# gooey-audio/libgooey

Measured on NVIDIA B200. Metric: voice-samples/sec, higher is better.
Workload: dtype f32

## Files before the change

libgooey_b200/csrc/kernels.cuh:

```cuda
#pragma once
#include <cuda_runtime.h>
#include "voices2.cuh"

namespace gd {

constexpr int TILE = 32;

template <class S> __device__ __forceinline__ void load_words(S& s, const uint32_t* base, int slot, int n_pad, int w0) {
  constexpr int W = sizeof(S) / 4;
  uint32_t* w = reinterpret_cast<uint32_t*>(&s);
#pragma unroll
  for (int i = 0; i < W; i++) w[i] = base[(size_t)(w0 + i) * n_pad + slot];
}
template <class S> __device__ __forceinline__ void store_words(const S& s, uint32_t* base, int slot, int n_pad, int w0) {
  constexpr int W = sizeof(S) / 4;
  const uint32_t* w = reinterpret_cast<const uint32_t*>(&s);
#pragma unroll
  for (int i = 0; i < W; i++) base[(size_t)(w0 + i) * n_pad + slot] = w[i];
}

struct KickV {
  using State = KickState; using Ctl = KickCtl; using Aud = KickAud; using Span = KickSpan;
  static constexpr bool FAST = true; static constexpr int NPL = KICK_PLANES;
  struct Run { KickDer d; int j_act; };
  static __device__ __forceinline__ float tick(State& s, const double* tt, const RateCtx& rc) { return kick_tick(s, tt, rc); }
  static __device__ __forceinline__ void slow_event(State& s, const VoiceEvent& e, const double* tt, const RateCtx&) {
    uint32_t r = 0; kick_event(s.c, e, tt, r); kick_span_begin(s.a, s.c, r);
  }
  static __device__ __forceinline__ bool settled(const Ctl& c) { return params_settled<K_NP>(c.cur, c.tgt); }
  static __device__ __forceinline__ void event(Ctl& c, const VoiceEvent& e, const double* tt, uint32_t& r) { kick_event(c, e, tt, r); }
  static __device__ __forceinline__ void plan(Ctl& c, uint32_t r, const double* tt, int ja, int jb, Span& sp) { kick_plan(c, r, tt, ja, jb, sp); }
  static __device__ __forceinline__ int front_end(const Span& sp) { return sp.j_act; }
  static __device__ __forceinline__ void front(const Span& sp, double now, uint32_t, float sr, float* o) {
    KickFront f = sp.d.drive <= 8.0f ? kick_front<true>(sp.c, sp.d, now, sr) : kick_front<false>(sp.c, sp.d, now, sr);
    o[0] = f.p1; o[1] = f.raw_click; o[2] = f.ne; o[3] = f.amp;
  }
  static __device__ __forceinline__ void span_begin(Aud& a, const Span& sp, Run& r, float) { kick_span_begin(a, sp.c, sp.resets); r.d = sp.d; r.j_act = sp.j_act; }
  static __device__ __forceinline__ void span_resume(const Span& sp, Run& r) { r.d = sp.d; r.j_act = sp.j_act; }
  static __device__ __forceinline__ bool wants_planes(const Aud&, const Run& r, int j) { return j < r.j_act; }
  static __device__ __forceinline__ bool is_active(const Aud&, const Run& r, int j) { return j < r.j_act; }
  static __device__ __forceinline__ float back(Aud& a, const Run& r, int j, const float* p, const RateCtx& rc) {
    if (j >= r.j_act) return 0.0f;
    KickFront f; f.p1 = p[0]; f.raw_click = p[1]; f.ne = p[2]; f.amp = p[3];
    return kick_back(a, r.d, f, rc);
  }
};
struct SnareV {
  using State = SnareState; using Ctl = SnareCtl; using Aud = SnareAud; using Span = SnareSpan;
  static constexpr bool FAST = true; static constexpr int NPL = SNARE_PLANES;
  struct Run { SnareDer d; int j_act; };
  static __device__ __forceinline__ float tick(State& s, const double* tt, const RateCtx& rc) { return snare_tick(s, tt, rc); }
  static __device__ __forceinline__ void slow_event(State& s, const VoiceEvent& e, const double* tt, const RateCtx&) {
    uint32_t r = 0; snare_event(s.c, e, tt, r); snare_span_begin(s.a, s.c, r);
  }
  static __device__ __forceinline__ bool settled(const Ctl& c) { return params_settled<S_NP>(c.cur, c.tgt); }
  static __device__ __forceinline__ void event(Ctl& c, const VoiceEvent& e, const double* tt, uint32_t& r) { snare_event(c, e, tt, r); }
  static __device__ __forceinline__ void plan(Ctl& c, uint32_t r, const double* tt, int ja, int jb, Span& sp) { snare_plan(c, r, tt, ja, jb, sp); }
  static __device__ __forceinline__ int front_end(const Span& sp) { return sp.j_act; }
  static __device__ __forceinline__ void front(const Span& sp, double now, uint32_t, float sr, float* o) {
    SnareFront f = snare_front<true>(sp.c, sp.d, now, sr);
    o[0] = f.tonal_out; o[1] = f.raw_noise; o[2] = f.cne; o[3] = f.crack_out; o[4] = f.amp;
  }
  static __device__ __forceinline__ void span_begin(Aud& a, const Span& sp, Run& r, float) { snare_span_begin(a, sp.c, sp.resets); r.d = sp.d; r.j_act = sp.j_act; }
  static __device__ __forceinline__ void span_resume(const Span& sp, Run& r) { r.d = sp.d; r.j_act = sp.j_act; }
  static __device__ __forceinline__ bool wants_planes(const Aud&, const Run& r, int j) { return j < r.j_act; }
  static __device__ __forceinline__ bool is_active(const Aud&, const Run& r, int j) { return j < r.j_act; }
  static __device__ __forceinline__ float back(Aud& a, const Run& r, int j, const float* p, const RateCtx& rc) {
    if (j >= r.j_act) return 0.0f;
    SnareFront f; f.tonal_out = p[0]; f.raw_noise = p[1]; f.cne = p[2]; f.crack_out = p[3]; f.amp = p[4];
    return snare_back(a, r.d, f, rc);
  }
};
struct HatV {
  using State = HatState; using Ctl = HatCtl; using Aud = HatAud; using Span = HatSpan;
  static constexpr bool FAST = true; static constexpr int NPL = HAT_PLANES;
  struct Run { HatDer d; int j_env; float env_final; };
  static __device__ __forceinline__ float tick(State& s, const double* tt, const RateCtx& rc) { return hat_tick(s, tt, rc); }
  static __device__ __forceinline__ void slow_event(State& s, const VoiceEvent& e, const double* tt, const RateCtx&) {
    uint32_t r = 0; hat_event(s.c, e, tt, r); hat_span_begin(s.a, s.c, r);
  }
  static __device__ __forceinline__ bool settled(const Ctl& c) { return params_settled<H_NP>(c.cur, c.tgt); }
  static __device__ __forceinline__ void event(Ctl& c, const VoiceEvent& e, const double* tt, uint32_t& r) { hat_event(c, e, tt, r); }
  static __device__ __forceinline__ void plan(Ctl& c, uint32_t r, const double* tt, int ja, int jb, Span& sp) { hat_plan(c, r, tt, ja, jb, sp); }
  static __device__ __forceinline__ int front_end(const Span& sp) { return sp.j_env < sp.j1 ? sp.j_env : sp.j1; }
  static __device__ __forceinline__ void front(const Span& sp, double now, uint32_t, float sr, float* o) { o[0] = hat_front(sp.c, sp.d, now, sr).env; }
  static __device__ __forceinline__ void span_begin(Aud& a, const Span& sp, Run& r, float) { hat_span_begin(a, sp.c, sp.resets); span_resume(sp, r); }
  static __device__ __forceinline__ void span_resume(const Span& sp, Run& r) { r.d = sp.d; r.j_env = sp.j_env; r.env_final = sp.env_final; }
  static __device__ __forceinline__ bool wants_planes(const Aud& a, const Run& r, int j) { return a.active && j < r.j_env; }
  static __device__ __forceinline__ bool is_active(const Aud& a, const Run&, int) { return a.active != 0; }
  static __device__ __forceinline__ float back(Aud& a, const Run& r, int j, const float* p, const RateCtx& rc) {
    if (!a.active) return 0.0f;
    HatFront f; f.env = j < r.j_env ? p[0] : r.env_final;
    return hat_back(a, r.d, f, j >= r.j_env, rc);
  }
};
struct TomV {
  using State = TomState; using Ctl = TomCtl; using Aud = TomAud; using Span = TomSpan;
  static constexpr bool FAST = true; static constexpr int NPL = TOM_PLANES;
  struct Run { TomDer d; int j_env; float env_final; };
  static __device__ __forceinline__ float tick(State& s, const double* tt, const RateCtx& rc) { return tom_tick(s, tt, rc); }
  static __device__ __forceinline__ void slow_event(State& s, const VoiceEvent& e, const double* tt, const RateCtx& rc) {
    uint32_t r = 0; tom_event(s.c, e, tt, r); tom_span_begin(s.a, s.c.mem_q_scale, s.c.mem_gain_scale, s.c.mem_dirty, r, rc.sr); s.c.mem_dirty = 0;
  }
  static __device__ __forceinline__ bool settled(const Ctl&) { return true; }
  static __device__ __forceinline__ void event(Ctl& c, const VoiceEvent& e, const double* tt, uint32_t& r) { tom_event(c, e, tt, r); }
  static __device__ __forceinline__ void plan(Ctl& c, uint32_t r, const double* tt, int ja, int jb, Span& sp) { tom_plan(c, r, tt, ja, jb, sp); }
  static __device__ __forceinline__ int front_end(const Span& sp) { return sp.d.membrane > 0.0f ? sp.j1 : (sp.j_env < sp.j1 ? sp.j_env + 1 : sp.j1); }
  static __device__ __forceinline__ void front(const Span& sp, double now, uint32_t k, float, float* o) {
    TomFront f = tom_front(sp.c, sp.d, now, k); o[0] = f.env; o[1] = f.noise; o[2] = f.rnd;
  }
  static __device__ __forceinline__ void span_begin(Aud& a, const Span& sp, Run& r, float sr) {
    tom_span_begin(a, sp.mem_q_scale, sp.mem_gain_scale, sp.mem_dirty, sp.resets, sr); span_resume(sp, r);
  }
// ... 64 lines not shown
      if (!((row_mask >> r) & 1u)) continue;
      const long long row = rows ? (long long)rows[r] : (long long)(row0 + r);
      if (lane < nf) out[row * stride + f0 + lane] = tile[r * 33 + lane];
    }
  }
}
__device__ __forceinline__ void load_tile_rows(float* tile , const float* plane, int pitch, int row0, int n_rows, int c0, int lane) {
  const int c = (lane & 7) * 4;
#pragma unroll
  for (int k = 0; k < 8; k++) {
    const int r = k * 4 + (lane >> 3);
    if (r < n_rows) {
      const float4 v = *reinterpret_cast<const float4*>(plane + (size_t)(row0 + r) * pitch + c0 + c);
      float* dst = tile + r * 33 + c;
      dst[0] = v.x; dst[1] = v.y; dst[2] = v.z; dst[3] = v.w;
    }
  }
}

__device__ __forceinline__ void load_tile_rows_any(float* tile , const float* plane, long long pitch, int row0, int n_rows, int c0, int nf, int lane) {
  for (int r = 0; r < n_rows; r++)
    if (lane < nf) tile[r * 33 + lane] = plane[(long long)(row0 + r) * pitch + c0 + lane];
}

template <class V, int BLOCK>
__global__ void __launch_bounds__(BLOCK) slow_kernel(const VoiceLaunch L) {
  __shared__ float tiles[BLOCK / 32][TILE * 33];
  const int v = blockIdx.x * BLOCK + threadIdx.x;
  const int lane = threadIdx.x & 31;
  const int warp = threadIdx.x >> 5;
// ... 144 lines not shown
#pragma unroll
        for (int q = 0; q < V::NPL; q++) p[q] = tl[q][lane * 33 + jj];
        tout[lane * 33 + jj] = V::back(a, run, j, p, L.rc);
      }
    }
    __syncwarp();
    store_tile_voice_major(tout, L.out, L.stride, L.row0 + warp_v0, L.rows ? L.rows + warp_v0 : nullptr, row_mask, L.chunk0 + f0, nf, lane);
    __syncwarp();
  }
  if (mine) {
    store_words(a, L.state, sv, L.n_pad, WC);
    L.span_cursor[v] = cur;
  }
}

#ifndef GOOEY_OWN_KERNELS_TU
__global__ void __launch_bounds__(64) lfo_kernel(LfoStream* __restrict__ streams, int n, float* __restrict__ planes, long long pitch, int frames) {
  const int i = blockIdx.x * blockDim.x + threadIdx.x;
  if (i >= n) return;
  LfoStream s = streams[i];
  float* out = s.plane >= 0 ? planes + (long long)s.plane * pitch : nullptr;
  for (int f = 0; f < frames; f++) {
    const float value = gm::g_sinf(s.phase * 2.0f * PI_F);
    s.phase += s.inc;
    if (s.phase >= 1.0f) s.phase -= 1.0f;
    if (out) out[f] = s.offset + (value * s.amount);
  }
  streams[i].phase = s.phase;
}
#endif
// ... 3 lines not shown
```

libgooey_b200/csrc/pool.cuh:

```cuda
#pragma once
#include <algorithm>
#include <atomic>
#include <map>
#include <type_traits>
#include <set>
#include <mutex>
#include "device_rt.h"
#include "wave.cuh"
#include "coop.cuh"
#include "gran_wave.cuh"
#include "bass_wave.cuh"
#include "poly_wave.cuh"
#include "../../include/gooey_batch.h"

namespace gh {

extern std::atomic<uint64_t> g_launches;

struct KernelStat { uint64_t launches = 0; double ms = 0.0; double voice_frames = 0.0; };
std::map<std::string, KernelStat>& kernel_stats();
std::mutex& kernel_stats_mutex();

__global__ void scatter_words_kernel(uint32_t* __restrict__ dst, long long cap, const uint32_t* __restrict__ src, const uint32_t* __restrict__ slots,
                                     int n, int words) {
// ... 135 lines not shown
  std::lock_guard<std::mutex> lk(mu);
  if (done.insert({dev, (const void*)kernel}).second)
    GH_CUDA(cudaFuncSetAttribute((const void*)kernel, cudaFuncAttributePreferredSharedMemoryCarveout, (int)cudaSharedmemCarveoutMaxShared));
}
#define GH_LAUNCH(kernel, grid, block, stream, ...) do { same_carveout(kernel); kernel<<<grid, block, 0, stream>>>(__VA_ARGS__); } while (0)

constexpr int CHUNK_FRAMES = 8192;
template <class V> struct TypeRunner {
  using State = typename V::State;
  Pool<State> pool;
  std::vector<uint32_t> slots, rows, ev_begin, span_off;
  std::vector<gd::VoiceEvent> ev_flat;
  std::vector<gd::ModRoute> routes_flat; std::vector<uint32_t> route_begin;
  DevBuf<gd::ModRoute> d_routes; DevBuf<uint32_t> d_route_begin;
  const float* mod_planes = nullptr; long long mod_pitch = 0; int mod_frame0 = 0;
  DevBuf<uint32_t> d_slots, d_rows, d_ev_begin, d_span_off, d_n_spans, d_span_cursor;
  DevBuf<gd::VoiceEvent> d_events;
  DevBuf<uint8_t> d_mode, d_spans;
  DevBuf<float> d_planes[2];
  cudaStream_t sB = nullptr, sC = nullptr, sS = nullptr;
  cudaEvent_t evA = nullptr, evB[2] = {nullptr, nullptr}, evC[2] = {nullptr, nullptr}, evDoneC = nullptr, evDoneS = nullptr;
  std::vector<cudaEvent_t> evT0, evT1;
  std::vector<double> timed_units;
  std::vector<cudaEvent_t> evChunk;
  int launched_chunks = 0;
  int timed_launches = 0;
  const char* backend_name = "back_kernel";
  static int chunk_of(int frames) { return std::min(CHUNK_FRAMES, (frames + 31) & ~31); }
  void wait_chunk(cudaStream_t s, int i) {
    if (n() == 0) return;
    if (launched_chunks == 0) { GH_CUDA(cudaStreamWaitEvent(s, evDoneC, 0)); return; }
    GH_CUDA(cudaStreamWaitEvent(s, evDoneS, 0));
    GH_CUDA(cudaStreamWaitEvent(s, evChunk[std::min(i, std::abs(launched_chunks) - 1)], 0));
  }

  int n() const { return (int)slots.size(); }
// ... 2 lines not shown
  void add(uint32_t slot, uint32_t out_row, const std::vector<gd::VoiceEvent>& events, const std::vector<gd::ModRoute>* routes = nullptr) {
    slots.push_back(slot); rows.push_back(out_row);
    if (routes) routes_flat.insert(routes_flat.end(), routes->begin(), routes->end());
    route_begin.push_back((uint32_t)routes_flat.size());
    uint32_t distinct = 0, last = 0xffffffffu;
    for (const auto& e : events) { if (e.frame != last) { distinct++; last = e.frame; } }
    ev_flat.insert(ev_flat.end(), events.begin(), events.end());
    ev_begin.push_back((uint32_t)ev_flat.size());
    span_off.push_back(span_off.back() + distinct + 1);
  }
  void ensure_streams() {
    if (sC) return;
    GH_CUDA(cudaStreamCreateWithFlags(&sB, cudaStreamNonBlocking));
    GH_CUDA(cudaStreamCreateWithFlags(&sC, cudaStreamNonBlocking));
    GH_CUDA(cudaStreamCreateWithFlags(&sS, cudaStreamNonBlocking));
    cudaEvent_t* evs[] = {&evA, &evB[0], &evB[1], &evC[0], &evC[1], &evDoneC, &evDoneS};
    for (auto e : evs) GH_CUDA(cudaEventCreateWithFlags(e, cudaEventDisableTiming));
  }
  ~TypeRunner() {
    cudaEvent_t evs[] = {evA, evB[0], evB[1], evC[0], evC[1], evDoneC, evDoneS};
    for (auto e : evs) if (e) cudaEventDestroy(e);
    for (auto e : evChunk) cudaEventDestroy(e);
    for (auto e : evT0) cudaEventDestroy(e);
    for (auto e : evT1) cudaEventDestroy(e);
    if (sB) cudaStreamDestroy(sB);
    if (sC) cudaStreamDestroy(sC);
    if (sS) cudaStreamDestroy(sS);
  }
  void collect_stats() {
    const char* name = backend_name;
    const int timed = V::FAST ? launched_chunks : timed_launches;
    if (timed <= 0) return;
    std::lock_guard<std::mutex> lk(kernel_stats_mutex());
    KernelStat& k = kernel_stats()[name];
    for (int i = 0; i < timed; i++) {
      float ms = 0.0f;
      if (cudaEventElapsedTime(&ms, evT0[i], evT1[i]) != cudaSuccess) { cudaGetLastError(); continue; }
      k.launches++; k.ms += ms; k.voice_frames += timed_units[i];
    }
    if (V::FAST) launched_chunks = -launched_chunks;
    else timed_launches = 0;
  }
// ... 13 lines not shown
    memset(&L, 0, sizeof L);
    L.state = pool.d.p; L.n = cnt; L.n_pad = pool.cap;
    L.slots = d_slots.p; L.rows = d_rows.p; L.row0 = 0;
    L.events = d_events.p; L.ev_begin = d_ev_begin.p; L.tt = tt; L.frames = frames; L.out = out; L.stride = stride; L.rc = rc;
    const bool modulated = !routes_flat.empty() && mod_planes;
    if (modulated) {
      d_routes.upload(routes_flat.data(), routes_flat.size(), sC);
      d_route_begin.upload(route_begin.data(), route_begin.size(), sC);
      L.routes = d_routes.p; L.route_begin = d_route_begin.p; L.mod_planes = mod_planes; L.mod_pitch = mod_pitch; L.mod_frame0 = mod_frame0;
    }
    if constexpr (V::FAST) {
      using Span = typename V::Span;
      d_span_off.upload(span_off.data(), span_off.size(), sC);
      d_n_spans.alloc(cnt); d_span_cursor.alloc(cnt); d_mode.alloc(cnt);
      d_spans.alloc((size_t)span_off.back() * sizeof(Span));
      const int chunk = chunk_of(frames);
      const int rows_pad = pad32(cnt);
      const size_t plane_floats = (size_t)rows_pad * chunk;
      d_planes[0].alloc(plane_floats * V::NPL); d_planes[1].alloc(plane_floats * V::NPL);
      L.mode = d_mode.p; L.spans = d_spans.p; L.span_off = d_span_off.p; L.n_spans = d_n_spans.p; L.span_cursor = d_span_cursor.p;
      L.plane_stride = (long long)plane_floats; L.pitch = chunk;
      GH_LAUNCH((gd::plan_kernel<V>), (cnt + 63) / 64, 64, sC, L);
      g_launches.fetch_add(1, std::memory_order_relaxed);
      GH_CUDA(cudaGetLastError());
      GH_CUDA(cudaEventRecord(evA, sC));
      GH_CUDA(cudaStreamWaitEvent(sB, evA, 0));
      GH_CUDA(cudaStreamWaitEvent(sS, evA, 0));
      GH_LAUNCH((gd::slow_kernel<V, 32>), (cnt + 31) / 32, 32, sS, L);
      g_launches.fetch_add(1, std::memory_order_relaxed);
      GH_CUDA(cudaGetLastError());
      GH_CUDA(cudaEventRecord(evDoneS, sS));
      const Back back = choose_back<V>(cnt);
      int i = 0;
      for (int c0 = 0; c0 < frames; c0 += chunk, i++) {
        const int b = i & 1;
        L.chunk0 = c0; L.chunk_frames = std::min(chunk, frames - c0);
        L.planes = d_planes[b].p;
        if (i >= 2) GH_CUDA(cudaStreamWaitEvent(sB, evC[b], 0));
        const int bpv = (L.chunk_frames + 255) / 256;
        GH_LAUNCH((gd::front_kernel<V, 256>), (unsigned)((size_t)cnt * bpv), 256, sB, L, bpv);
        GH_CUDA(cudaGetLastError());
        GH_CUDA(cudaEventRecord(evB[b], sB));
        GH_CUDA(cudaStreamWaitEvent(sC, evB[b], 0));
        if ((int)evT0.size() <= i) { cudaEvent_t e0, e1; GH_CUDA(cudaEventCreate(&e0)); GH_CUDA(cudaEventCreate(&e1)); evT0.push_back(e0); evT1.push_back(e1); timed_units.push_back(0.0); }
        timed_units[i] = (double)cnt * L.chunk_frames;
        GH_CUDA(cudaEventRecord(evT0[i], sC));
        switch (back) {
          case Back::Coop:
            if constexpr (std::is_same<V, gd::TomV>::value) coop_launch(cnt, sC, L);
            backend_name = "coop_kernel<TomC>";
            break;
          case Back::Wave:
            GH_LAUNCH((gd::wave::wave_kernel<typename WaveOf<V>::W>), cnt, 32, sC, L);
            backend_name = WaveOf<V>::name;
            break;
          case Back::Serial:
            GH_LAUNCH((gd::back_kernel<V, 32>), (cnt + 31) / 32, 32, sC, L);
// ... 71 lines not shown
```

libgooey_b200/csrc/voices.cuh:

```cuda
#pragma once
#include "dsp.cuh"
#include "events.h"

namespace gd {

struct RateCtx {
  float sr;
  double dt;
  float smooth15;
  float smooth10, smooth30, smooth50;
  float click_alpha;
  float asym_down;
  PinkCoef pink;
};
G_HD RateCtx make_rate_ctx(float sr) {
  RateCtx c;
  c.sr = sr;
  c.dt = 1.0 / (double)sr;
  c.smooth15 = smooth_coeff(sr, 15.0f);
  c.smooth10 = smooth_coeff(sr, 10.0f);
  c.smooth30 = smooth_coeff(sr, 30.0f);
  c.smooth50 = smooth_coeff(sr, 50.0f);
  c.click_alpha = 1.0f - gm::g_expf(-2.0f * PI_F * 8000.0f / sr);
  c.asym_down = 1.0f - gm::g_expf(-1.0f / 100.0f);
// ... 485 lines not shown
  else { je = (jd < 0 ? ja : jd) + 1; if (je > jb) je = jb; c.active = 0; }
  sp.j_act = je;
  c.k += (uint32_t)(jb - ja);
}

enum { H_PITCH, H_DECAY, H_ATTACK, H_TONE, H_VOLUME, H_TUNING, H_NP };
struct HatCtl {
  float cur[H_NP], tgt[H_NP];
  uint32_t pink_on, db24;
  MaxEnv2 env;
  float velocity;
  uint32_t k;
};
struct HatAud {
  float mod_phase, main_phase, env_smooth;
  uint32_t active;
  Biquad hp1, hp2;
  Tpt svf;
  uint64_t white;
  Pink pink;
};
struct HatState { HatCtl c; HatAud a; };
struct HatDer { float pitch_hz, tone_hz, vel035, volume; uint32_t pink_on, db24; MaxEnvK ek; };
struct HatFront { float env; };
enum { HAT_PLANES = 1 };
G_HD float hat_pitch_hz(float p) { return denorm(p * p, 3500.0f, 10000.0f); }

G_HD void hat_init(HatState& s, const float* cfg, uint32_t pink_on, uint32_t db24, float sr) {
  HatCtl& c = s.c; HatAud& a = s.a;
  for (int i = 0; i < 5; i++) { float v = clampf(cfg[i], 0.0f, 1.0f); c.cur[i] = c.tgt[i] = v; }
  c.cur[H_TUNING] = c.tgt[H_TUNING] = 0.5f;
  c.pink_on = pink_on; c.db24 = db24;
  c.env.target[0] = c.env.target[1] = 0; c.env.dur[0] = c.env.dur[1] = 0; c.env.curve[0] = c.env.curve[1] = 0;
  c.env.seg_start = 0.0; c.env.seg_start_val = 0; c.env.cur_val = 0; c.env.seg = 2; c.env.active = 0;
  c.velocity = 1.0f; c.k = 0;
  a.mod_phase = a.main_phase = 0.0f; a.env_smooth = 0.0f; a.active = 0;
  hp_init(a.hp1, sr); hp_init(a.hp2, sr);
  tpt_init(a.svf, sr, denorm(c.cur[H_TONE], 500.0f, 10000.0f), 0.5f);
  a.white = XS_SEED;
  pink_reset(a.pink);
}
G_HD void hat_trigger(HatCtl& c, float velocity, double time) {
  c.velocity = clampf(velocity, 0.0f, 1.0f);
  float attack_ms = denorm(c.cur[H_ATTACK], 0.5f, 200.0f);
  float decay_ms = denorm(c.cur[H_DECAY], 0.5f, 4000.0f);
  maxenv_init(c.env, 1.0f, attack_ms, -0.3f, 0.0f, decay_ms, -0.8f);
  maxenv_trigger(c.env, time);
}
G_HD void hat_event(HatCtl& c, const VoiceEvent& e, const double* tt, uint32_t& resets) {
  switch (e.kind) {
    case EV_TRIGGER: hat_trigger(c, e.value, tt[c.k]); resets |= RST_TRIGGER; break;
// ... 348 lines not shown
```

libgooey_b200/csrc/wave.cuh:

```cuda
#pragma once
#include "kernels.cuh"

namespace gd { namespace wave {

__device__ __forceinline__ float shup(float v, int d) { return __shfl_up_sync(0xffffffffu, v, d); }
__device__ __forceinline__ float shl(float v, int n) { return __shfl_sync(0xffffffffu, v, n); }
__device__ __forceinline__ bool gall(bool p) { return __all_sync(0xffffffffu, p); }
__device__ __forceinline__ unsigned gballot(bool p) { return __ballot_sync(0xffffffffu, p); }
__device__ __forceinline__ void gsync() { __syncwarp(); }

struct Geo1 { float m[5]; float ap; };
struct Geo2 { float a; float m[5]; float ap; };

__device__ __forceinline__ Geo1 make_geo1(float a, int lane) {
  Geo1 g; float p = a, ap = 1.0f; const int e = lane + 1;
#pragma unroll
  for (int i = 0; i < 5; i++) { g.m[i] = lane >= (1 << i) ? p : 0.0f; if (e & (1 << i)) ap *= p; p *= p; }
  if (e & 32) ap *= p;
  g.ap = ap;
  return g;
}
__device__ __forceinline__ Geo2 make_geo2(float a, int lane) {
  Geo2 g; g.a = a; float p = a * a, ap = 1.0f;
#pragma unroll
// ... 147 lines not shown

__device__ __forceinline__ float w_tanh(float x) {
  const float ax = fabsf(x);
  const float e = __expf(2.0f * ax);
  const float t = 1.0f - __fdividef(2.0f, e + 1.0f);
  return copysignf(t, x);
}
__device__ __forceinline__ float w_gain_comp(FbShaper& w, float env) {
  const float reference = fmaxf(env, 0.05f);
  const float driven = fmaxf(fabsf(w_tanh(reference * w.drive)), 1e-6f);
  const float comp_no_fb = w_tanh(reference) / driven;
  const float makeup = fbws_makeup(w);
  const float taming = 1.0f / (1.0f + comp_no_fb * w.feedback * 0.25f);
  return fminf(comp_no_fb * taming * makeup, 3.0f);
}
__device__ __forceinline__ float wrap01(float x) { return x < 1.0f ? x : (x < 2.0f ? x - 1.0f : fmodf(x, 1.0f)); }

struct TptLin { float in0, in1; };
__device__ __forceinline__ TptLin tpt_lin_init(Lin2& S, const Tpt& f, int lane) {
  const float g = f.g, h = f.h, gh = g * h, g2h = g * gh;
  lin2_init(S, 2.0f * h - 1.0f, -2.0f * gh, 2.0f * gh, 1.0f - 2.0f * g2h, lane);
  TptLin t; t.in0 = 2.0f * gh; t.in1 = 2.0f * g2h;
  return t;
}
__device__ __forceinline__ void tpt_scan(const Lin2& S, const TptLin& t, Tpt& f, float in, float& ic1_pre, float& ic2_pre, int lane, int last) {
  float s0 = t.in0 * in, s1 = t.in1 * in;
  lin2_scan(S, s0, s1, f.ic1, f.ic2, lane);
  ic1_pre = prev_lane(s0, f.ic1, lane); ic2_pre = prev_lane(s1, f.ic2, lane);
  f.ic1 = shl(s0, last); f.ic2 = shl(s1, last);
}
__device__ __forceinline__ void biquad_lin_init(Lin2& S, const Biquad& b, int lane) { lin2_init(S, -b.a1, -b.a2, 1.0f, 0.0f, lane); }
// ... 11 lines not shown

#define LANE_VAL(v, n) shl((v), (n))
#define STASH_PUT(slot, v) (sc.stash[slot][lane] = (v))
#define STASH_GET(slot, n) (sc.stash[slot][n])

struct KickW {
  using V = KickV;
  struct Span2 { bool noise, shaper, serial; };
  static __device__ __forceinline__ int active_end(const KickV::Run& r) { return r.j_act; }
  static __device__ __forceinline__ void span_setup(KickAud& a, const KickV::Run& r, Span2& w, WaveScratch&, const RateCtx& rc, int) {
    w.noise = r.d.noise_amount > 0.001f;
    a.ws.drive = r.d.drive; a.ws.feedback = r.d.feedback;
    fbws_set_cutoff(a.ws, rc.sr, r.d.fb_cutoff);
    w.shaper = !(a.ws.mix <= 0.0001f || a.ws.drive <= 1.0f);
    w.serial = w.shaper && a.ws.feedback != 0.0f;
    if (w.noise) rlp_set(a.noise_lp, rc.sr, r.d.noise_cut, r.d.noise_res);
  }
  static __device__ __forceinline__ float block(KickAud& a, const KickV::Run& r, const Span2& w, WaveScratch& sc, const GeoTables& T,
                                                const float* p, int, int& nl, const RateCtx& rc, int lane) {
    const int last = nl - 1;
    const float p1 = p[0], raw_click = p[1], ne = p[2], amp = p[3];
    float hp_l = 0.0f, fn_l = 0.0f;
    gsync(); STASH_PUT(0, raw_click); gsync();
#pragma unroll 4
    for (int n = 0; n < nl; n++) {
      const float raw = STASH_GET(0, n);
      const float hp = raw - a.click_hp;
      a.click_hp += rc.click_alpha * hp;
      float fn = 0.0f;
      if (w.noise) fn = rlp_process(a.noise_lp, pink_tick(a.pink, rc.pink));
      if (n == lane) { hp_l = hp; fn_l = fn; }
    }
    const float filt_click = hp_l * (1.0f + 4.0f * 0.1f);
    const float noise_out = w.noise ? fn_l * ne * r.d.noise_amount * 0.5f : 0.0f;
    const float total = p1 + filt_click + noise_out;
    float od = total;
    const bool finite = gall(isfinite(total));
    if (w.serial || (w.shaper && !finite)) {
#pragma unroll 4
      for (int n = 0; n < nl; n++) {
        const float y = fbws_process(a.ws, LANE_VAL(total, n));
        if (n == lane) od = y;
      }
    } else if (w.shaper) {
      FbShaper& ws = a.ws;
      const float fb_in = ws.drive * total + ws.feedback * ws.last_out;
      const float shaped = os_scan(ws.os, fb_in, [](float x) { return w_tanh(x); }, T, lane, last);
// ... 21 lines not shown
        ws.filter_state += ws.filter_coeff * (out - ws.filter_state);
        if (fabsf(ws.filter_state) < 1e-15f) ws.filter_state = 0.0f;
        if (n == lane) out_l = out;
      }
      ws.last_out = ws.filter_state;
      od = total * (1.0f - ws.mix) + out_l * ws.mix;
    }
    return od * amp * r.d.va * r.d.volume;
  }
};

struct SnareW {
  using V = SnareV;
  struct Span2 { float comp; bool shaper; };
  static __device__ __forceinline__ int active_end(const SnareV::Run& r) { return r.j_act; }
  static __device__ __forceinline__ void span_setup(SnareAud& a, const SnareV::Run& r, Span2& w, WaveScratch&, const RateCtx& rc, int) {
    chamb_set(a.filt, rc.sr, r.d.cutoff, r.d.res);
    a.ws.drive = r.d.drive;
    w.shaper = !(a.ws.mix <= 0.0001f || a.ws.drive <= 1.0f);
    w.comp = w.shaper ? gm::g_tanhf(0.5f) / gm::g_tanhf(0.5f * a.ws.drive) : 1.0f;
  }
  static __device__ __forceinline__ float block(SnareAud& a, const SnareV::Run& r, const Span2& w, WaveScratch& sc, const GeoTables& T,
                                                const float* p, int, int& nl, const RateCtx&, int lane) {
    const int last = nl - 1;
    const float tonal_out = p[0], raw_noise = p[1], cne = p[2], crack_out = p[3], amp = p[4];
    float low_l = 0.0f, band_l = 0.0f, high_l = 0.0f;
    {
      const float f = a.filt.f, q = a.filt.q;
      float low = a.filt.low, band = a.filt.band;
      gsync(); STASH_PUT(0, raw_noise); gsync();
#pragma unroll 4
      for (int n = 0; n < nl; n++) {
        const float in = STASH_GET(0, n);
        float high = 0.0f;
#pragma unroll
        for (int i = 0; i < 2; i++) { low = low + f * band; high = in - low - q * band; band = f * high + band; }
        if (n == lane) { low_l = low; band_l = band; high_l = high; }
      }
      a.filt.low = low; a.filt.band = band;
    }
    const float filtered = svf_pick(low_l, band_l, high_l, r.d.filter_type);
    const float noise_out = filtered * cne * r.d.noise_mix;
    const float total = tonal_out + noise_out + crack_out;
    float od = total;
    const bool finite = gall(isfinite(total));
    if (!finite) {
#pragma unroll 4
      for (int n = 0; n < nl; n++) {
        const float y = ws_process(a.ws, LANE_VAL(total, n));
        if (n == lane) od = y;
      }
    } else if (w.shaper) {
      const float d = a.ws.drive, comp = w.comp;
      const float sat = os_scan(a.ws.os, total, [d, comp](float x) { return w_tanh(x * d) * comp; }, T, lane, last);
      od = total * (1.0f - a.ws.mix) + sat * a.ws.mix;
    }
// ... 1 lines not shown
  }
};

struct HatW {
  using V = HatV;
  struct Span2 { TptLin svf; };
  static __device__ __forceinline__ int active_end(const HatV::Run&) { return 0x7fffffff; }
  static __device__ __forceinline__ void span_setup(HatAud& a, const HatV::Run& r, Span2& w, WaveScratch& sc, const RateCtx& rc, int lane) {
    hp_set(a.hp1, rc.sr, r.d.pitch_hz, 1.0f);
    biquad_lin_init(sc.lin[0], a.hp1, lane);
    if (r.d.db24) { hp_set(a.hp2, rc.sr, r.d.pitch_hz, 1.0f); biquad_lin_init(sc.lin[1], a.hp2, lane); }
    tpt_set(a.svf, rc.sr, r.d.tone_hz, 0.5f);
    w.svf = tpt_lin_init(sc.lin[2], a.svf, lane);
  }
  static __device__ __forceinline__ float block(HatAud& a, const HatV::Run& r, const Span2& w, WaveScratch& sc, const GeoTables&,
                                                const float* p, int j, int& nl, const RateCtx& rc, int lane) {
    const float sr = rc.sr;
    const float env_l = (j + lane) < r.j_env ? p[0] : r.env_final;
    float es_l = 0.0f;
    int nv = nl;
    gsync(); STASH_PUT(0, env_l); gsync();
    if (j + nl <= r.j_env) {
#pragma unroll 4
      for (int n = 0; n < nl; n++) {
        const float e = STASH_GET(0, n);
        if (e >= a.env_smooth) a.env_smooth = e; else a.env_smooth += rc.asym_down * (e - a.env_smooth);
        if (n == lane) es_l = a.env_smooth;
      }
    } else {
#pragma unroll 4
      for (int n = 0; n < nl; n++) {
        const float e = STASH_GET(0, n);
        if (e >= a.env_smooth) a.env_smooth = e; else a.env_smooth += rc.asym_down * (e - a.env_smooth);
        if (n == lane) es_l = a.env_smooth;
        if ((j + n) >= r.j_env && a.env_smooth < 1e-4f) { nv = n + 1; a.active = 0; break; }
      }
    }
    nl = nv;
    float noise = 0.0f, mph = 0.0f, nph = 0.0f;
    const float inc_mod = fmaxf(r.d.pitch_hz * 0.1f, 0.0f) / sr, inc_main = fmaxf(r.d.pitch_hz, 0.0f) / sr;
    const bool small_inc = inc_main < 1.0f && a.mod_phase < 1.0f && a.main_phase < 1.0f;
    if (!r.d.pink_on && small_inc) {
      uint64_t st_l = 0;
#pragma unroll 4
      for (int n = 0; n < nv; n++) {
        uint64_t x = a.white;
        x ^= x >> 12; x ^= x << 25; x ^= x >> 27;
        a.white = x;
        float pm = a.mod_phase + inc_mod; a.mod_phase = pm < 1.0f ? pm : pm - 1.0f;
        float pn = a.main_phase + inc_main; a.main_phase = pn < 1.0f ? pn : pn - 1.0f;
        if (n == lane) { st_l = x; mph = a.mod_phase; nph = a.main_phase; }
      }
      const float u = u64_to_f32(st_l * 0x2545f4914f6cdd1dull) / 18446744073709551616.0f;
      noise = (u * 2.0f) - 1.0f;
    } else {
#pragma unroll 4
      for (int n = 0; n < nv; n++) {
        float x;
        if (r.d.pink_on) x = pink_tick(a.pink, rc.pink);
        else { float u = u64_to_f32(xorshift64s_next(a.white)) / 18446744073709551616.0f; x = (u * 2.0f) - 1.0f; }
        a.mod_phase = wrap01(a.mod_phase + inc_mod);
        a.main_phase = wrap01(a.main_phase + inc_main);
        if (n == lane) { noise = x; mph = a.mod_phase; nph = a.main_phase; }
      }
    }
    float ph = mph + noise * 0.25f; ph -= floorf(ph);
    const float mod_out = gm::g_sinf(2.0f * PI_F * ph);
    ph = nph + mod_out * 0.75f; ph -= floorf(ph);
    const float main_out = gm::g_sinf(2.0f * PI_F * ph);
    const int last = nv - 1;
    float filtered = biquad_scan(sc.lin[0], a.hp1, main_out, lane, last);
    if (r.d.db24) filtered = biquad_scan(sc.lin[1], a.hp2, filtered, lane, last) * 0.8f;
    const float out = filtered * es_l * r.d.vel035 * 0.35f;
    float ic1p, ic2p;
    tpt_scan(sc.lin[2], w.svf, a.svf, out, ic1p, ic2p, lane, last);
    const float v1 = (a.svf.g * (out - ic2p) + ic1p) * a.svf.h;
    const float v2 = ic2p + a.svf.g * v1;
    const float hi = out - (a.svf.r * v1 + v2);
    return hi * r.d.volume;
  }
// ... 180 lines not shown
      mem_out = membrane(a, sc, filtered * env_l, nv, lane);
      gsync(); STASH_PUT(5, fabsf(mem_out) * 0.001f); gsync();
#pragma unroll 4
      for (int n = 0; n < nv; n++) a.ring_level = a.ring_level * 0.999f + STASH_GET(5, n);
    }
    const float dry_gain = 1.0f - d.mm;
    const float dry = filtered * env_l;
    const float fs = dry * dry_gain + mem_out * d.mm;
    return fs * fade * 0.7f * d.vol;
  }
};

template <class W>
__global__ void __launch_bounds__(32, 1) wave_kernel(const VoiceLaunch L) {
  using V = typename W::V; using Span = typename V::Span; using Aud = typename V::Aud;
  constexpr int WC = sizeof(typename V::Ctl) / 4;
  __shared__ GeoTables T;
  __shared__ WaveScratch sc;
  const int lane = threadIdx.x & 31;
  geo_tables_init(T, L.rc, threadIdx.x, 32);
  __syncthreads();
  const int v = blockIdx.x;
  const bool alive = v < L.n && L.mode[v] == 0;
  const int sv = alive ? (L.slots ? (int)L.slots[v] : v) : 0;
  Aud a;
  const Span* spans = nullptr;
  uint32_t ns = 0, cur = 0xffffffffu;
  typename V::Run run;
  typename W::Span2 w2;
  bool ready = false;
  int next_j0 = 0x7fffffff;
  float* out = nullptr;
  const float* planes = nullptr;
  if (alive) {
    load_words(a, L.state, sv, L.n_pad, WC);
    spans = reinterpret_cast<const Span*>(L.spans) + L.span_off[v];
    ns = L.n_spans[v];
    cur = L.span_cursor[v];
    if (cur != 0xffffffffu) V::span_resume(spans[cur], run);
    next_j0 = cur + 1u < ns ? spans[cur + 1u].j0 : 0x7fffffff;
    const long long row = L.rows ? (long long)L.rows[v] : (long long)(L.row0 + v);
    out = L.out + row * L.stride;
    planes = L.planes + (size_t)v * L.pitch;
  }
  const int c1 = L.chunk0 + min(L.chunk_frames, L.frames - L.chunk0);
  int j = L.chunk0;
  while (alive && j < c1) {
    while (j == next_j0) {
      cur += 1u;
      V::span_begin(a, spans[cur], run, L.rc.sr);
      ready = false;
      next_j0 = cur + 1u < ns ? spans[cur + 1u].j0 : 0x7fffffff;
    }
    const int span_end = min(next_j0, c1);
    const int act_end = min(span_end, W::active_end(run));
    if (cur == 0xffffffffu || !V::is_active(a, run, j) || j >= act_end) {
      for (int k = j + lane; k < span_end; k += 32) out[k] = 0.0f;
      j = span_end;
      continue;
    }
    if (!ready) { gsync(); W::span_setup(a, run, w2, sc, L.rc, lane); ready = true; }
    int nl = min(32, act_end - j);
    float p[V::NPL];
    const int jj = j + min(lane, nl - 1);
#pragma unroll
    for (int q = 0; q < V::NPL; q++) p[q] = planes[(size_t)q * L.plane_stride + (jj - L.chunk0)];
    const float y = W::block(a, run, w2, sc, T, p, j, nl, L.rc, lane);
    if (lane < nl) out[j + lane] = y;
    j += nl;
  }
  if (alive && lane == 0) {
    store_words(a, L.state, sv, L.n_pad, WC);
    L.span_cursor[v] = cur;
  }
}

#undef LANE_VAL
} }
```

Before: 8.861 billion.

## Split serial per-sample recurrences into replay kernel on high-priority stream

Moves the sequential per-sample recurrences (kick click HP and noise LP, snare SVF, hat envelope smoothing, noise and phase accumulators) out of the warp-wide wave kernel into a new replay kernel. In that kernel each lane owns one voice and walks its samples through shared-memory tiles. The results are written as extra planes that the wave kernel reads directly, removing the 32-step warp-serial loops and their syncs. The replay kernel runs on a separate high-priority stream between the front and wave stages. This adds plane memory traffic, an extra launch per chunk, and a state-struct split, including a reordered HatAud layout.

Result: slower. 7.125 billion, median of 6 (-19.6%).

```diff
diff --git a/libgooey_b200/csrc/kernels.cuh b/libgooey_b200/csrc/kernels.cuh
--- a/libgooey_b200/csrc/kernels.cuh
+++ b/libgooey_b200/csrc/kernels.cuh
@@ -18,6 +18,18 @@
 #pragma unroll
   for (int i = 0; i < W; i++) base[(size_t)(w0 + i) * n_pad + slot] = w[i];
 }
+template <int I0, int I1, class S> __device__ __forceinline__ void load_word_range(S& s, const uint32_t* base, int slot, int n_pad, int w0) {
+  uint32_t* w = reinterpret_cast<uint32_t*>(&s);
+#pragma unroll
+  for (int i = I0; i < I1; i++) w[i] = base[(size_t)(w0 + i) * n_pad + slot];
+}
+template <int I0, int I1, class S> __device__ __forceinline__ void store_word_range(const S& s, uint32_t* base, int slot, int n_pad, int w0) {
+  const uint32_t* w = reinterpret_cast<const uint32_t*>(&s);
+#pragma unroll
+  for (int i = I0; i < I1; i++) base[(size_t)(w0 + i) * n_pad + slot] = w[i];
+}
+
+__device__ __forceinline__ float wrap01(float x) { return x < 1.0f ? x : (x < 2.0f ? x - 1.0f : fmodf(x, 1.0f)); }
 
 struct KickV {
   using State = KickState; using Ctl = KickCtl; using Aud = KickAud; using Span = KickSpan;
@@ -44,6 +56,22 @@
     KickFront f; f.p1 = p[0]; f.raw_click = p[1]; f.ne = p[2]; f.amp = p[3];
     return kick_back(a, r.d, f, rc);
   }
+  static constexpr int NRP = 2, R_IN = 1, R_WORDS = offsetof(KickAud, ws) / 4;
+  struct RSpan { bool noise; };
+  static __device__ __forceinline__ int replay_until(const Run& r) { return r.j_act; }
+  static __device__ __forceinline__ void replay_begin(Aud&, const uint32_t*, int, bool) {}
+  static __device__ __forceinline__ void replay_end(Aud&) {}
+  static __device__ __forceinline__ void replay_setup(Aud& a, const Run& r, RSpan& s, const RateCtx& rc) {
+    s.noise = r.d.noise_amount > 0.001f;
+    if (s.noise) rlp_set(a.noise_lp, rc.sr, r.d.noise_cut, r.d.noise_res);
+  }
+  static __device__ __forceinline__ void replay(Aud& a, const Run&, const RSpan& s, int, float raw_click, const RateCtx& rc, float* o) {
+    const float hp = raw_click - a.click_hp;
+    a.click_hp += rc.click_alpha * hp;
+    float fn = 0.0f;
+    if (s.noise) fn = rlp_process(a.noise_lp, pink_tick(a.pink, rc.pink));
+    o[0] = hp; o[1] = fn;
+  }
 };
 struct SnareV {
   using State = SnareState; using Ctl = SnareCtl; using Aud = SnareAud; using Span = SnareSpan;
@@ -69,6 +97,15 @@
     if (j >= r.j_act) return 0.0f;
     SnareFront f; f.tonal_out = p[0]; f.raw_noise = p[1]; f.cne = p[2]; f.crack_out = p[3]; f.amp = p[4];
     return snare_back(a, r.d, f, rc);
+  }
+  static constexpr int NRP = 1, R_IN = 1, R_WORDS = offsetof(SnareAud, ws) / 4;
+  struct RSpan {};
+  static __device__ __forceinline__ int replay_until(const Run& r) { return r.j_act; }
+  static __device__ __forceinline__ void replay_begin(Aud&, const uint32_t*, int, bool) {}
+  static __device__ __forceinline__ void replay_end(Aud&) {}
+  static __device__ __forceinline__ void replay_setup(Aud& a, const Run& r, RSpan&, const RateCtx& rc) { chamb_set(a.filt, rc.sr, r.d.cutoff, r.d.res); }
+  static __device__ __forceinline__ void replay(Aud& a, const Run& r, const RSpan&, int, float raw_noise, const RateCtx&, float* o) {
+    o[0] = chamb_process(a.filt, raw_noise, r.d.filter_type);
   }
 };
 struct HatV {
@@ -93,10 +130,32 @@
     HatFront f; f.env = j < r.j_env ? p[0] : r.env_final;
     return hat_back(a, r.d, f, j >= r.j_env, rc);
   }
+  static constexpr int NRP = 4, R_IN = 0, R_WORDS = offsetof(HatAud, active) / 4;
+  struct RSpan { float inc_mod, inc_main; };
+  static __device__ __forceinline__ int replay_until(const Run&) { return 0x7fffffff; }
+  static __device__ __forceinline__ void replay_begin(Aud& a, const uint32_t* aud, int n_pad, bool call_start) {
+    a.active = call_start ? aud[(size_t)(offsetof(HatAud, active) / 4) * n_pad] : a.r_active;
+  }
+  static __device__ __forceinline__ void replay_end(Aud& a) { a.r_active = a.active; }
+  static __device__ __forceinline__ void replay_setup(Aud&, const Run& r, RSpan& s, const RateCtx& rc) {
+    s.inc_mod = fmaxf(r.d.pitch_hz * 0.1f, 0.0f) / rc.sr; s.inc_main = fmaxf(r.d.pitch_hz, 0.0f) / rc.sr;
+  }
+  static __device__ __forceinline__ void replay(Aud& a, const Run& r, const RSpan& s, int j, float env, const RateCtx& rc, float* o) {
+    const float e = j < r.j_env ? env : r.env_final;
+    if (e >= a.env_smooth) a.env_smooth = e; else a.env_smooth += rc.asym_down * (e - a.env_smooth);
+    float x;
+    if (r.d.pink_on) x = pink_tick(a.pink, rc.pink);
+    else { float u = u64_to_f32(xorshift64s_next(a.white)) / 18446744073709551616.0f; x = (u * 2.0f) - 1.0f; }
+    a.mod_phase = wrap01(a.mod_phase + s.inc_mod);
+    a.main_phase = wrap01(a.main_phase + s.inc_main);
+    o[0] = a.env_smooth; o[1] = x; o[2] = a.mod_phase; o[3] = a.main_phase;
+    if (j >= r.j_env && a.env_smooth < 1e-4f) a.active = 0;
+  }
 };
 struct TomV {
   using State = TomState; using Ctl = TomCtl; using Aud = TomAud; using Span = TomSpan;
   static constexpr bool FAST = true; static constexpr int NPL = TOM_PLANES;
+  static constexpr int NRP = 0, R_WORDS = 0;
   struct Run { TomDer d; int j_env; float env_final; };
   static __device__ __forceinline__ float tick(State& s, const double* tt, const RateCtx& rc) { return tom_tick(s, tt, rc); }
   static __device__ __forceinline__ void slow_event(State& s, const VoiceEvent& e, const double* tt, const RateCtx& rc) {
@@ -191,6 +250,18 @@
       const float4 v = *reinterpret_cast<const float4*>(plane + (size_t)(row0 + r) * pitch + c0 + c);
       float* dst = tile + r * 33 + c;
       dst[0] = v.x; dst[1] = v.y; dst[2] = v.z; dst[3] = v.w;
+    }
+  }
+}
+
+__device__ __forceinline__ void store_tile_rows(const float* tile , float* plane, int pitch, int row0, int n_rows, int c0, int lane) {
+  const int c = (lane & 7) * 4;
+#pragma unroll
+  for (int k = 0; k < 8; k++) {
+    const int r = k * 4 + (lane >> 3);
+    if (r < n_rows) {
+      const float* src = tile + r * 33 + c;
+      *reinterpret_cast<float4*>(plane + (size_t)(row0 + r) * pitch + c0 + c) = make_float4(src[0], src[1], src[2], src[3]);
     }
   }
 }
@@ -365,6 +436,86 @@
   }
 }
 
+template <class V>
+__global__ void __launch_bounds__(32) replay_kernel(const VoiceLaunch L, uint32_t* __restrict__ cursor) {
+  using Span = typename V::Span; using Aud = typename V::Aud;
+  constexpr int WC = sizeof(typename V::Ctl) / 4;
+  __shared__ float tiles[1 + V::NRP][TILE * 33];
+  const int lane = threadIdx.x;
+  const int warp_v0 = blockIdx.x * 32;
+  const int v = warp_v0 + lane;
+  const bool mine = v < L.n && L.mode[v] == 0;
+  if (__ballot_sync(0xffffffffu, mine) == 0) return;
+  const int n_rows = min(32, L.n - warp_v0);
+  Aud a;
+  typename V::Run run;
+  typename V::RSpan rs;
+  bool ready = false;
+  const Span* spans = nullptr;
+  uint32_t cur = 0xffffffffu, ns = 0;
+  int next_j0 = 0x7fffffff;
+  int sv = v;
+  if (mine) {
+    if (L.slots) sv = (int)L.slots[v];
+    load_word_range<0, V::R_WORDS>(a, L.state, sv, L.n_pad, WC);
+    V::replay_begin(a, L.state + (size_t)WC * L.n_pad + sv, L.n_pad, L.chunk0 == 0);
+    spans = reinterpret_cast<const Span*>(L.spans) + L.span_off[v];
+    ns = L.n_spans[v];
+    if (L.chunk0 > 0) cur = cursor[v];
+    if (cur != 0xffffffffu) V::span_resume(spans[cur], run);
+    const uint32_t nx = cur + 1u;
+    next_j0 = nx < ns ? spans[nx].j0 : 0x7fffffff;
+  }
+  float* tin = tiles[0];
+  const int cend = min(L.chunk_frames, L.frames - L.chunk0);
+  for (int f0 = 0; f0 < cend; f0 += TILE) {
+    const int nf = min(TILE, cend - f0);
+    bool want = false;
+    if (mine) want = V::wants_planes(a, run, L.chunk0 + f0) || next_j0 < L.chunk0 + f0 + nf;
+    if (__any_sync(0xffffffffu, want)) load_tile_rows(tin, L.planes + (size_t)V::R_IN * L.plane_stride, L.pitch, warp_v0, n_rows, f0, lane);
+    __syncwarp();
+    if (mine) {
+      const int t0 = L.chunk0 + f0;
+      int jj = 0;
+      while (jj < nf) {
+        while (t0 + jj == next_j0) {
+          cur += 1u;
+          V::span_begin(a, spans[cur], run, L.rc.sr);
+          ready = false;
+          next_j0 = cur + 1u < ns ? spans[cur + 1u].j0 : 0x7fffffff;
+        }
+        const int seg = min(nf, next_j0 - t0);
+        int k = jj;
+        if (cur != 0xffffffffu && V::is_active(a, run, t0 + k)) {
+          if (!ready) { V::replay_setup(a, run, rs, L.rc); ready = true; }
+          const int e = min(seg, V::replay_until(run) - t0);
+#pragma unroll 4
+          for (; k < e && V::is_active(a, run, t0 + k); k++) {
+            float o[V::NRP];
+            V::replay(a, run, rs, t0 + k, tin[lane * 33 + k], L.rc, o);
+#pragma unroll
+            for (int q = 0; q < V::NRP; q++) tiles[1 + q][lane * 33 + k] = o[q];
+          }
+        }
+        for (; k < seg; k++) {
+#pragma unroll
+          for (int q = 0; q < V::NRP; q++) tiles[1 + q][lane * 33 + k] = 0.0f;
+        }
+        jj = seg;
+      }
+    }
+    __syncwarp();
+#pragma unroll
+    for (int q = 0; q < V::NRP; q++) store_tile_rows(tiles[1 + q], L.planes + (size_t)(V::NPL + q) * L.plane_stride, L.pitch, warp_v0, n_rows, f0, lane);
+    __syncwarp();
+  }
+  if (mine) {
+    V::replay_end(a);
+    store_word_range<0, V::R_WORDS>(a, L.state, sv, L.n_pad, WC);
+    cursor[v] = cur;
+  }
+}
+
 #ifndef GOOEY_OWN_KERNELS_TU
 __global__ void __launch_bounds__(64) lfo_kernel(LfoStream* __restrict__ streams, int n, float* __restrict__ planes, long long pitch, int frames) {
   const int i = blockIdx.x * blockDim.x + threadIdx.x;
diff --git a/libgooey_b200/csrc/pool.cuh b/libgooey_b200/csrc/pool.cuh
--- a/libgooey_b200/csrc/pool.cuh
+++ b/libgooey_b200/csrc/pool.cuh
@@ -173,12 +173,12 @@
   std::vector<gd::ModRoute> routes_flat; std::vector<uint32_t> route_begin;
   DevBuf<gd::ModRoute> d_routes; DevBuf<uint32_t> d_route_begin;
   const float* mod_planes = nullptr; long long mod_pitch = 0; int mod_frame0 = 0;
-  DevBuf<uint32_t> d_slots, d_rows, d_ev_begin, d_span_off, d_n_spans, d_span_cursor;
+  DevBuf<uint32_t> d_slots, d_rows, d_ev_begin, d_span_off, d_n_spans, d_span_cursor, d_replay_cursor;
   DevBuf<gd::VoiceEvent> d_events;
   DevBuf<uint8_t> d_mode, d_spans;
   DevBuf<float> d_planes[2];
-  cudaStream_t sB = nullptr, sC = nullptr, sS = nullptr;
-  cudaEvent_t evA = nullptr, evB[2] = {nullptr, nullptr}, evC[2] = {nullptr, nullptr}, evDoneC = nullptr, evDoneS = nullptr;
+  cudaStream_t sB = nullptr, sC = nullptr, sS = nullptr, sR = nullptr;
+  cudaEvent_t evA = nullptr, evF[2] = {nullptr, nullptr}, evB[2] = {nullptr, nullptr}, evC[2] = {nullptr, nullptr}, evDoneC = nullptr, evDoneS = nullptr;
   std::vector<cudaEvent_t> evT0, evT1;
   std::vector<double> timed_units;
   std::vector<cudaEvent_t> evChunk;
@@ -211,11 +211,14 @@
     GH_CUDA(cudaStreamCreateWithFlags(&sB, cudaStreamNonBlocking));
     GH_CUDA(cudaStreamCreateWithFlags(&sC, cudaStreamNonBlocking));
     GH_CUDA(cudaStreamCreateWithFlags(&sS, cudaStreamNonBlocking));
-    cudaEvent_t* evs[] = {&evA, &evB[0], &evB[1], &evC[0], &evC[1], &evDoneC, &evDoneS};
+    int least = 0, greatest = 0;
+    GH_CUDA(cudaDeviceGetStreamPriorityRange(&least, &greatest));
+    GH_CUDA(cudaStreamCreateWithPriority(&sR, cudaStreamNonBlocking, greatest));
+    cudaEvent_t* evs[] = {&evA, &evF[0], &evF[1], &evB[0], &evB[1], &evC[0], &evC[1], &evDoneC, &evDoneS};
     for (auto e : evs) GH_CUDA(cudaEventCreateWithFlags(e, cudaEventDisableTiming));
   }
   ~TypeRunner() {
-    cudaEvent_t evs[] = {evA, evB[0], evB[1], evC[0], evC[1], evDoneC, evDoneS};
+    cudaEvent_t evs[] = {evA, evF[0], evF[1], evB[0], evB[1], evC[0], evC[1], evDoneC, evDoneS};
     for (auto e : evs) if (e) cudaEventDestroy(e);
     for (auto e : evChunk) cudaEventDestroy(e);
     for (auto e : evT0) cudaEventDestroy(e);
@@ -223,6 +226,7 @@
     if (sB) cudaStreamDestroy(sB);
     if (sC) cudaStreamDestroy(sC);
     if (sS) cudaStreamDestroy(sS);
+    if (sR) cudaStreamDestroy(sR);
   }
   void collect_stats() {
     const char* name = backend_name;
@@ -266,10 +270,14 @@
       d_span_off.upload(span_off.data(), span_off.size(), sC);
       d_n_spans.alloc(cnt); d_span_cursor.alloc(cnt); d_mode.alloc(cnt);
       d_spans.alloc((size_t)span_off.back() * sizeof(Span));
+      const Back back = choose_back<V>(cnt);
+      const bool replay = back == Back::Wave && V::NRP > 0;
+      if (replay) d_replay_cursor.alloc(cnt);
       const int chunk = chunk_of(frames);
       const int rows_pad = pad32(cnt);
       const size_t plane_floats = (size_t)rows_pad * chunk;
-      d_planes[0].alloc(plane_floats * V::NPL); d_planes[1].alloc(plane_floats * V::NPL);
+      const int n_planes = V::NPL + (replay ? V::NRP : 0);
+      d_planes[0].alloc(plane_floats * n_planes); d_planes[1].alloc(plane_floats * n_planes);
       L.mode = d_mode.p; L.spans = d_spans.p; L.span_off = d_span_off.p; L.n_spans = d_n_spans.p; L.span_cursor = d_span_cursor.p;
       L.plane_stride = (long long)plane_floats; L.pitch = chunk;
       GH_LAUNCH((gd::plan_kernel<V>), (cnt + 63) / 64, 64, sC, L);
@@ -282,7 +290,6 @@
       g_launches.fetch_add(1, std::memory_order_relaxed);
       GH_CUDA(cudaGetLastError());
       GH_CUDA(cudaEventRecord(evDoneS, sS));
-      const Back back = choose_back<V>(cnt);
       int i = 0;
       for (int c0 = 0; c0 < frames; c0 += chunk, i++) {
         const int b = i & 1;
@@ -292,7 +299,18 @@
         const int bpv = (L.chunk_frames + 255) / 256;
         GH_LAUNCH((gd::front_kernel<V, 256>), (unsigned)((size_t)cnt * bpv), 256, sB, L, bpv);
         GH_CUDA(cudaGetLastError());
-        GH_CUDA(cudaEventRecord(evB[b], sB));
+        cudaStream_t sPlanes = sB;
+        if constexpr (V::NRP > 0) {
+          if (replay) {
+            GH_CUDA(cudaEventRecord(evF[b], sB));
+            GH_CUDA(cudaStreamWaitEvent(sR, evF[b], 0));
+            GH_LAUNCH((gd::replay_kernel<V>), (cnt + 31) / 32, 32, sR, L, d_replay_cursor.p);
+            GH_CUDA(cudaGetLastError());
+            g_launches.fetch_add(1, std::memory_order_relaxed);
+            sPlanes = sR;
+          }
+        }
+        GH_CUDA(cudaEventRecord(evB[b], sPlanes));
         GH_CUDA(cudaStreamWaitEvent(sC, evB[b], 0));
         if ((int)evT0.size() <= i) { cudaEvent_t e0, e1; GH_CUDA(cudaEventCreate(&e0)); GH_CUDA(cudaEventCreate(&e1)); evT0.push_back(e0); evT1.push_back(e1); timed_units.push_back(0.0); }
         timed_units[i] = (double)cnt * L.chunk_frames;
diff --git a/libgooey_b200/csrc/voices.cuh b/libgooey_b200/csrc/voices.cuh
--- a/libgooey_b200/csrc/voices.cuh
+++ b/libgooey_b200/csrc/voices.cuh
@@ -523,11 +523,12 @@
 };
 struct HatAud {
   float mod_phase, main_phase, env_smooth;
+  uint32_t r_active;
+  uint64_t white;
+  Pink pink;
   uint32_t active;
   Biquad hp1, hp2;
   Tpt svf;
-  uint64_t white;
-  Pink pink;
 };
 struct HatState { HatCtl c; HatAud a; };
 struct HatDer { float pitch_hz, tone_hz, vel035, volume; uint32_t pink_on, db24; MaxEnvK ek; };
@@ -543,7 +544,7 @@
   c.env.target[0] = c.env.target[1] = 0; c.env.dur[0] = c.env.dur[1] = 0; c.env.curve[0] = c.env.curve[1] = 0;
   c.env.seg_start = 0.0; c.env.seg_start_val = 0; c.env.cur_val = 0; c.env.seg = 2; c.env.active = 0;
   c.velocity = 1.0f; c.k = 0;
-  a.mod_phase = a.main_phase = 0.0f; a.env_smooth = 0.0f; a.active = 0;
+  a.mod_phase = a.main_phase = 0.0f; a.env_smooth = 0.0f; a.active = a.r_active = 0;
   hp_init(a.hp1, sr); hp_init(a.hp2, sr);
   tpt_init(a.svf, sr, denorm(c.cur[H_TONE], 500.0f, 10000.0f), 0.5f);
   a.white = XS_SEED;
diff --git a/libgooey_b200/csrc/wave.cuh b/libgooey_b200/csrc/wave.cuh
--- a/libgooey_b200/csrc/wave.cuh
+++ b/libgooey_b200/csrc/wave.cuh
@@ -185,7 +185,6 @@
   const float taming = 1.0f / (1.0f + comp_no_fb * w.feedback * 0.25f);
   return fminf(comp_no_fb * taming * makeup, 3.0f);
 }
-__device__ __forceinline__ float wrap01(float x) { return x < 1.0f ? x : (x < 2.0f ? x - 1.0f : fmodf(x, 1.0f)); }
 
 struct TptLin { float in0, in1; };
 __device__ __forceinline__ TptLin tpt_lin_init(Lin2& S, const Tpt& f, int lane) {
@@ -227,23 +226,12 @@
     fbws_set_cutoff(a.ws, rc.sr, r.d.fb_cutoff);
     w.shaper = !(a.ws.mix <= 0.0001f || a.ws.drive <= 1.0f);
     w.serial = w.shaper && a.ws.feedback != 0.0f;
-    if (w.noise) rlp_set(a.noise_lp, rc.sr, r.d.noise_cut, r.d.noise_res);
   }
   static __device__ __forceinline__ float block(KickAud& a, const KickV::Run& r, const Span2& w, WaveScratch& sc, const GeoTables& T,
                                                 const float* p, int, int& nl, const RateCtx& rc, int lane) {
     const int last = nl - 1;
-    const float p1 = p[0], raw_click = p[1], ne = p[2], amp = p[3];
-    float hp_l = 0.0f, fn_l = 0.0f;
-    gsync(); STASH_PUT(0, raw_click); gsync();
-#pragma unroll 4
-    for (int n = 0; n < nl; n++) {
-      const float raw = STASH_GET(0, n);
-      const float hp = raw - a.click_hp;
-      a.click_hp += rc.click_alpha * hp;
-      float fn = 0.0f;
-      if (w.noise) fn = rlp_process(a.noise_lp, pink_tick(a.pink, rc.pink));
-      if (n == lane) { hp_l = hp; fn_l = fn; }
-    }
+    const float p1 = p[0], ne = p[2], amp = p[3];
+    const float hp_l = p[KICK_PLANES], fn_l = p[KICK_PLANES + 1];
     const float filt_click = hp_l * (1.0f + 4.0f * 0.1f);
     const float noise_out = w.noise ? fn_l * ne * r.d.noise_amount * 0.5f : 0.0f;
     const float total = p1 + filt_click + noise_out;
@@ -295,8 +283,7 @@
   using V = SnareV;
   struct Span2 { float comp; bool shaper; };
   static __device__ __forceinline__ int active_end(const SnareV::Run& r) { return r.j_act; }
-  static __device__ __forceinline__ void span_setup(SnareAud& a, const SnareV::Run& r, Span2& w, WaveScratch&, const RateCtx& rc, int) {
-    chamb_set(a.filt, rc.sr, r.d.cutoff, r.d.res);
+  static __device__ __forceinline__ void span_setup(SnareAud& a, const SnareV::Run& r, Span2& w, WaveScratch&, const RateCtx&, int) {
     a.ws.drive = r.d.drive;
     w.shaper = !(a.ws.mix <= 0.0001f || a.ws.drive <= 1.0f);
     w.comp = w.shaper ? gm::g_tanhf(0.5f) / gm::g_tanhf(0.5f * a.ws.drive) : 1.0f;
@@ -304,23 +291,8 @@
   static __device__ __forceinline__ float block(SnareAud& a, const SnareV::Run& r, const Span2& w, WaveScratch& sc, const GeoTables& T,
                                                 const float* p, int, int& nl, const RateCtx&, int lane) {
     const int last = nl - 1;
-    const float tonal_out = p[0], raw_noise = p[1], cne = p[2], crack_out = p[3], amp = p[4];
-    float low_l = 0.0f, band_l = 0.0f, high_l = 0.0f;
-    {
-      const float f = a.filt.f, q = a.filt.q;
-      float low = a.filt.low, band = a.filt.band;
-      gsync(); STASH_PUT(0, raw_noise); gsync();
-#pragma unroll 4
-      for (int n = 0; n < nl; n++) {
-        const float in = STASH_GET(0, n);
-        float high = 0.0f;
-#pragma unroll
-        for (int i = 0; i < 2; i++) { low = low + f * band; high = in - low - q * band; band = f * high + band; }
-        if (n == lane) { low_l = low; band_l = band; high_l = high; }
-      }
-      a.filt.low = low; a.filt.band = band;
-    }
-    const float filtered = svf_pick(low_l, band_l, high_l, r.d.filter_type);
+    const float tonal_out = p[0], cne = p[2], crack_out = p[3], amp = p[4];
+    const float filtered = p[SNARE_PLANES];
     const float noise_out = filtered * cne * r.d.noise_mix;
     const float total = tonal_out + noise_out + crack_out;
     float od = total;
@@ -352,56 +324,12 @@
     w.svf = tpt_lin_init(sc.lin[2], a.svf, lane);
   }
   static __device__ __forceinline__ float block(HatAud& a, const HatV::Run& r, const Span2& w, WaveScratch& sc, const GeoTables&,
-                                                const float* p, int j, int& nl, const RateCtx& rc, int lane) {
-    const float sr = rc.sr;
-    const float env_l = (j + lane) < r.j_env ? p[0] : r.env_final;
-    float es_l = 0.0f;
-    int nv = nl;
-    gsync(); STASH_PUT(0, env_l); gsync();
-    if (j + nl <= r.j_env) {
-#pragma unroll 4
-      for (int n = 0; n < nl; n++) {
-        const float e = STASH_GET(0, n);
-        if (e >= a.env_smooth) a.env_smooth = e; else a.env_smooth += rc.asym_down * (e - a.env_smooth);
-        if (n == lane) es_l = a.env_smooth;
-      }
-    } else {
-#pragma unroll 4
-      for (int n = 0; n < nl; n++) {
-        const float e = STASH_GET(0, n);
-        if (e >= a.env_smooth) a.env_smooth = e; else a.env_smooth += rc.asym_down * (e - a.env_smooth);
-        if (n == lane) es_l = a.env_smooth;
-        if ((j + n) >= r.j_env && a.env_smooth < 1e-4f) { nv = n + 1; a.active = 0; break; }
-      }
-    }
-    nl = nv;
-    float noise = 0.0f, mph = 0.0f, nph = 0.0f;
-    const float inc_mod = fmaxf(r.d.pitch_hz * 0.1f, 0.0f) / sr, inc_main = fmaxf(r.d.pitch_hz, 0.0f) / sr;
-    const bool small_inc = inc_main < 1.0f && a.mod_phase < 1.0f && a.main_phase < 1.0f;
-    if (!r.d.pink_on && small_inc) {
-      uint64_t st_l = 0;
-#pragma unroll 4
-      for (int n = 0; n < nv; n++) {
-        uint64_t x = a.white;
-        x ^= x >> 12; x ^= x << 25; x ^= x >> 27;
-        a.white = x;
-        float pm = a.mod_phase + inc_mod; a.mod_phase = pm < 1.0f ? pm : pm - 1.0f;
-        float pn = a.main_phase + inc_main; a.main_phase = pn < 1.0f ? pn : pn - 1.0f;
-        if (n == lane) { st_l = x; mph = a.mod_phase; nph = a.main_phase; }
-      }
-      const float u = u64_to_f32(st_l * 0x2545f4914f6cdd1dull) / 18446744073709551616.0f;
-      noise = (u * 2.0f) - 1.0f;
-    } else {
-#pragma unroll 4
-      for (int n = 0; n < nv; n++) {
-        float x;
-        if (r.d.pink_on) x = pink_tick(a.pink, rc.pink);
-        else { float u = u64_to_f32(xorshift64s_next(a.white)) / 18446744073709551616.0f; x = (u * 2.0f) - 1.0f; }
-        a.mod_phase = wrap01(a.mod_phase + inc_mod);
-        a.main_phase = wrap01(a.main_phase + inc_main);
-        if (n == lane) { noise = x; mph = a.mod_phase; nph = a.main_phase; }
-      }
-    }
+                                                const float* p, int j, int& nl, const RateCtx&, int lane) {
+    const float es_l = p[HAT_PLANES], noise = p[HAT_PLANES + 1], mph = p[HAT_PLANES + 2], nph = p[HAT_PLANES + 3];
+    const unsigned valid = nl >= 32 ? 0xffffffffu : ((1u << nl) - 1u);
+    const unsigned off = gballot((j + lane) >= r.j_env && es_l < 1e-4f) & valid;
+    if (off) { nl = __ffs(off); a.active = 0; }
+    const int nv = nl;
     float ph = mph + noise * 0.25f; ph -= floorf(ph);
     const float mod_out = gm::g_sinf(2.0f * PI_F * ph);
     ph = nph + mod_out * 0.75f; ph -= floorf(ph);
@@ -612,7 +540,8 @@
 template <class W>
 __global__ void __launch_bounds__(32, 1) wave_kernel(const VoiceLaunch L) {
   using V = typename W::V; using Span = typename V::Span; using Aud = typename V::Aud;
-  constexpr int WC = sizeof(typename V::Ctl) / 4;
+  constexpr int WC = sizeof(typename V::Ctl) / 4, AW = sizeof(Aud) / 4;
+  constexpr int NP = V::NPL + V::NRP;
   __shared__ GeoTables T;
   __shared__ WaveScratch sc;
   const int lane = threadIdx.x & 31;
@@ -631,7 +560,7 @@
   float* out = nullptr;
   const float* planes = nullptr;
   if (alive) {
-    load_words(a, L.state, sv, L.n_pad, WC);
+    load_word_range<V::R_WORDS, AW>(a, L.state, sv, L.n_pad, WC);
     spans = reinterpret_cast<const Span*>(L.spans) + L.span_off[v];
     ns = L.n_spans[v];
     cur = L.span_cursor[v];
@@ -659,16 +588,16 @@
     }
     if (!ready) { gsync(); W::span_setup(a, run, w2, sc, L.rc, lane); ready = true; }
     int nl = min(32, act_end - j);
-    float p[V::NPL];
+    float p[NP];
     const int jj = j + min(lane, nl - 1);
 #pragma unroll
-    for (int q = 0; q < V::NPL; q++) p[q] = planes[(size_t)q * L.plane_stride + (jj - L.chunk0)];
+    for (int q = 0; q < NP; q++) p[q] = planes[(size_t)q * L.plane_stride + (jj - L.chunk0)];
     const float y = W::block(a, run, w2, sc, T, p, j, nl, L.rc, lane);
     if (lane < nl) out[j + lane] = y;
     j += nl;
   }
   if (alive && lane == 0) {
-    store_words(a, L.state, sv, L.n_pad, WC);
+    store_word_range<V::R_WORDS, AW>(a, L.state, sv, L.n_pad, WC);
     L.span_cursor[v] = cur;
   }
 }
```
